# PecanProject/sipnet

Measured on AMD Instinct MI355X. Metric: ensemble-site-timesteps/sec, higher is better.
Workload: dtype f64; 1 GPU; c10k: 1 site(s) x 10240 members per GPU x 17520 half-hourly steps, perturbed params, default flags; sites_per_gpu=1, fast_math=True, gather=n/a (1 GPU), parallelism=ensemble-sharded x1, ranks_seen=1, devices_seen=1, kernel=stepCoopKernel<double, true, true, false>

## Files before the change

### sipnet_amd/csrc/coop_wave_carbon.inc

```

  COOP_CODE_PHASE(0);
  const R K_invLcsw = (R)(1.0 / PRM(leafCSpWt));
  const R K_wtr = (R)PRM(woodTurnoverRate), K_ltr = (R)PRM(leafTurnoverRate);
  const R K_frt = (R)PRM(fineRootTurnoverRate), K_crt = (R)PRM(coarseRootTurnoverRate);
  const R K_la = (R)PRM(leafAllocation), K_wa = (R)PRM(woodAllocation);
  const R K_fa = (R)PRM(fineRootAllocation), K_ca = (R)PRM(coarseRootAllocation);
  const double gddLeafOn = PRM(gddLeafOn);
  const double leafOffDay = PRM(leafOffDay) > 0 ? PRM(leafOffDay) : 1e300;

  const R G_iLeafCN = NCyc ? (R)(1.0 / PRM(leafCN)) : R(0), G_iWoodCN = NCyc ? (R)(1.0 / PRM(woodCN)) : R(0);
  const R G_iFineCN = NCyc ? (R)(1.0 / PRM(fineRootCN)) : R(0), G_resorbC = NCyc ? (R)PRM(leafNResorptionFrac) : R(0);
  const double G_nVolD = NCyc ? PRM(nVolatilizationFrac) : 0.0, G_nLeachD = NCyc ? PRM(nLeachingFrac) : 0.0;
  double plantWoodC = ST(plantWoodC), plantLeafC = ST(plantLeafC), soilC = NCyc ? 0.0 : ST(soilC);
  double coarseRootC = ST(coarseRootC), fineRootC = ST(fineRootC);
  const R X_growthFrac = F_growthResp ? (R)PRM(growthRespFrac) : R(0);
  const R X_lbrK = F_litterPool ? (R)(PRM(litterBreakdownRate) / PRM(baseSoilResp)) : R(0);
  const R X_flr = Opt ? (R)PRM(fracLitterRespired) : R(0), X_1mFlr = Opt ? (R)(1.0 - PRM(fracLitterRespired)) : R(0);
  const R X_soilCH4 = F_anaerobic ? (R)PRM(soilMethaneRate) : R(0);
  const R X_litCH4 = (F_anaerobic && F_litterPool) ? (R)PRM(litterMethaneRate) : R(0);
  const R X_iSoilCSat = (Opt && F_carbonSat) ? (R)(1.0 / PRM(soilCSaturation)) : R(0);
  double litterC = Opt ? ST(litterC) : 0.0;
  auto optSoilSide = [&](R eSoilC, R eLitter, R soilCNow, R fSoil, R qSoilT, R mK, R rootLoss, R aboveLitter, R len,
                         R& rSoil, R& rHet, double& soilGain, double& litterGain, R& methane) {
#pragma clang fp contract(off)
    rSoil = eSoilC * fSoil;
    const R breakdown = eLitter * (X_lbrK * fSoil);
    const R rLitter = breakdown * X_flr, litterToSoil = breakdown * X_1mFlr;
    const R qm = qSoilT * mK;
    const R soilMethane = X_soilCH4 * eSoilC * qm, litterMethane = X_litCH4 * eLitter * qm;
    const R sat = clip01(soilCNow * X_iSoilCSat);
    const R soilInputs = rootLoss + litterToSoil;
    const R dLitter = aboveLitter + soilInputs * sat - litterToSoil - rLitter - litterMethane;
    const R dSoilTwo = soilInputs * (R(1) - sat) - rSoil - soilMethane;
    const R dSoilOne = rootLoss + aboveLitter - rSoil - soilMethane;
// ... 64 lines not shown
                     fineRootCreation * G_iFineCN);
    const R nDemand = plantNDemand();
    postD(&mailPlant[t & 1][0][lane], 0, (double)leafLitter);
    postD(&mailPlant[t & 1][0][lane], 1, (double)woodLitter);
    postD(&mailPlant[t & 1][0][lane], 2, (double)fineRootLoss);
    postD(&mailPlant[t & 1][0][lane], 3, (double)coarseRootLoss);
    postD(&mailPlant[t & 1][0][lane], 4, (double)nDemand);
    postD(&mailPlant[t & 1][0][lane], 5, (double)reductionN);
    postD(&mailPlant[t & 1][0][lane], 6, (double)leafOnN(leafOnCreation + evLeafOnAll));
    postD(&mailPlant[t & 1][0][lane], 7, (double)leafOnN(leafOnCreation));
    postFlag(&seqPlant, t);
    if (__builtin_expect(minNSeq < t, 0)) {
      WAIT_BEGIN()
      takeD1(&mailMinN[t & 1][lane], &seqMinN, t, minNStep);
      WAIT_END(2)
    }
    if (__builtin_expect(__builtin_amdgcn_ballot_w64(!nPlentiful(minNStep, qSoilD, lenD, G_nVolD, G_nLeachD, (double)nDemand)) != 0, 0)) {
      double sAvail, sFixFrac, sUnclaimed;
      takeD3(&mailSupply[0][lane], &seqSupply, t, sAvail, sFixFrac, sUnclaimed);
      const R availableMinN = (R)sAvail, fixFrac = (R)sFixFrac, unclaimed = (R)sUnclaimed;
      const R nUptake = (R(1) - fixFrac) * rmax0(nDemand - unclaimed * invLen);
      const R uptakeDemand = nUptake * len;
      const bool limited = uptakeDemand > R(kTiny) && uptakeDemand > availableMinN;
      const R red = limited ? fdiv(fdiv(availableMinN, R(1) - fixFrac) + unclaimed, nDemand * len) : R(1);
      woodCreation *= red;
      leafCreation *= red;
      fineRootCreation *= red;
      coarseRootCreation *= red;
      postD(&mailDemand[0][lane], 0, (double)plantNDemand());
      postFlag(&seqDemand, t);
    }
  };

  for (int tileStart = curTile * kFastTile; tileStart < tEnd; tileStart += kFastTile, curTile++) {
    if constexpr (Sums) {
      if (tileStart > tBegin) {
        if (RingLds) asm volatile("s_waitcnt vmcnt(0)" ::: "memory");
        else asm volatile("s_waitcnt vmcnt(1)" ::: "memory");
      }
    } else {
    if (tileStart > tBegin) {
      if (RingLds) asm volatile("s_waitcnt vmcnt(1)" ::: "memory");
      else asm volatile("s_waitcnt vmcnt(2)" ::: "memory");
    }
    }
    stageTile(curTile + 1, (curTile + 1) & 1);
    const int tFirst = tileStart > tBegin ? tileStart : tBegin;
    const int tLast = (tileStart + kFastTile) < tEnd ? (tileStart + kFastTile) : tEnd;
    const unsigned char* recB = lds + (curTile & 1) * kTileBytes +
                                (int)(tFirst - tileFirst(curTile)) * (int)sizeof(FastRec);
    int t = tFirst;
    if (!Full && ringClean && !(a.options & SIPNET_KOPT_NO_REGULAR_TILES)) {
      d2 h0, h7;
      i4 hj;
      double hW1, hEndGdd, hEndDay;
      int hTile;
      asm volatile("ds_read_b128 %0, %7\n\tds_read_b128 %1, %7 offset:112\n\tds_read_b128 %2, %7 offset:128\n\t"
                   "ds_read_b64 %3, %7 offset:144\n\tds_read_b32 %4, %7 offset:208\n\tds_read_b64 %5, %7 offset:216\n\t"
                   "ds_read_b64 %6, %7 offset:224\n\ts_waitcnt lgkmcnt(0)"
                   : "=&v"(h0), "=&v"(h7), "=&v"(hj), "=&v"(hW1), "=&v"(hTile), "=&v"(hEndGdd), "=&v"(hEndDay)
                   : "v"(ldsAddr(recB)) : "memory");
      const int tileBits = uni(hTile);
      const bool phenSafe = (allOn || hEndGdd < minGddOn) && (allOff || hEndDay < minOffDay);
      if ((tileBits & FAST_TILE_REGULAR) && __builtin_amdgcn_ballot_w64(!phenSafe) == 0) {
        const R len = (R)h0.x, invLen = (R)h0.y;
        const int nOps = uni(hj.x) >> 16;
        const int slots0 = uni(hj.y);
        auto nextSlot = [](int s) { return s + 1 == SIPNET_RING_SLOTS ? 0 : s + 1; };
        const double wA = nOps == 2 ? h7.y : 0.0, wB = nOps == 2 ? hW1 : h7.y;
        int readSlot = nOps == 2 ? ((slots0 >> 8) & 255) : (slots0 & 255);
        int insSlot = uni(hj.z);
        double vPrev = 0.0;
        if (nOps == 2) {
          const int s0 = slots0 & 255;
          vPrev = RingLds ? ringL[s0 * 64 + lane] : (s0 == lastIns ? lastNpp : (double)ringp[(uint32_t)s0 * ncu]);
        }
        R photosynthesis = 0, rSoil = 0, rVeg = 0, rCoarseRoot = 0, rFineRoot = 0, rHet = 0;
        [[maybe_unused]] R methaneReg = 0;
        double soilGain = 0.0, litterGain = 0.0, ringNew = 0.0;
        R rvN = 0;
        bool rootsOk = true, useLast = false, dyingStep = false;
        auto finishStep = [&](auto mayDie) {
#pragma clang fp contract(off)
          constexpr bool MayDie = decltype(mayDie)::value;
          bool diedNow = false;
          double deathToSoil0 = 0.0, deathToSoil1 = 0.0;
          if (MayDie) ringClean = false;
          if (MayDie && !(rootsOk && (plantWoodC + delta > kTiny))) {
            aliveC = false;
            diedNow = true;
            if (diedAt < 0) diedAt = t;
            deathToSoil0 = fineRootC + coarseRootC;
            deathToSoil1 = plantWoodC + plantLeafC + delta;
            if (NCyc) {
              postD(&mailDeath[0][lane], 0, deathToSoil0);
              postD(&mailDeath[0][lane], 1, deathToSoil1);
              postD(&mailDeath[0][lane], 2, fineRootC * (double)G_iFineCN + coarseRootC * (double)G_iWoodCN);
              postD(&mailDeath[0][lane], 3, plantWoodC * (double)G_iWoodCN + plantLeafC * (double)G_iLeafCN);
            }
            plantWoodC = 0.0;
            plantLeafC = 0.0;
            coarseRootC = 0.0;
            fineRootC = 0.0;
            delta = 0.0;
            ringSum = 0.0;
          }
          plantWoodC = rmax0(plantWoodC);
          plantLeafC = rmax0(plantLeafC);
          coarseRootC = rmax0(coarseRootC);
          fineRootC = rmax0(fineRootC);
          const R tGpp = photosynthesis * len;
          const R tRa = ffma(rVeg, len, (rCoarseRoot + rFineRoot) * len);
          if (NCyc) postD(&mailPend[t & 1][0][lane], 0, (double)(tGpp - tRa));
          postAlive(&mailAlive[(t + 1) & 1][lane], t + 1, diedNow);
          if (!NCyc) {
            soilC += soilGain;
            if (Opt) litterC += litterGain;
            if (MayDie && diedNow) {
              soilC += deathToSoil0;
              if (Opt && F_litterPool) litterC += deathToSoil1;
              else soilC += deathToSoil1;
            }
            soilC = rmax0(soilC);
            if (Opt) litterC = rmax0(litterC);
          }
          const R tRh = (Opt ? rHet : rSoil) * len;
          const R tNee = R(-1.0) * ((tGpp - tRa) - tRh);
          if (!NCyc) totNee += (double)tNee;
          const double npp = (double)(photosynthesis - rVeg - rCoarseRoot - rFineRoot);
          if (!RingLds) asm volatile("s_waitcnt vmcnt(0)" : "+v"(rvN) :: "memory");
          const double vNew = RingLds ? ringNew : (useLast ? lastNpp : (double)rvN);
          if (!(MayDie && diedNow)) {
            ringSum = ffma(-wA, vPrev, ringSum);
            ringSum = ffma(-wB, vNew, ringSum);
            ringSum = ffma(npp, (double)len, ringSum);
          } else {
            ringValidFrom = t + 1;
          }
          vPrev = vNew;
          if (RingLds) {
            ringL[insSlot * 64 + lane] = npp;
          } else {
            ringp[(uint32_t)insSlot * ncu] = (R)npp;
            lastIns = insSlot;
            lastNpp = npp;
          }
          if constexpr (Sums && !NCyc) {
            sumsC.nee += (double)tNee;
            if (--sumsC.left == 0) {
              *oNee = (OutT)sumsC.nee;
              oNee += ldNee;
              sumsC.nee = 0.0;
              sumsC.left = a.sumEvery;
            }
          } else {
          if (!NCyc) {
            *oNee = tNee;
            oNee += ldNee;
          }
          }
          if (__builtin_expect(stageOn, 0)) postRaw(&stage[0][(t - tBegin) & (2 * kStageR - 1)][lane], tNee);
        };
        unsigned dayMask = ((unsigned)tileBits >> 16) >> (t - tileStart);
        for (; t < tLast; t++, dayMask >>= 1) {
#pragma clang fp contract(off)
          MARK("C regular step begin")
          R g1, g2, qSoilT, gFine, gCoarse, moistEff;
          R mK = 0;
          ringNew = 0.0;
          double minNStep = 0.0;
          int minNSeq = 0;
          {
            WAIT_BEGIN()
            if (NCyc)
              takeFactorsN(&mailFac[t & 1][0][lane], &seqFac, &mailMinN[t & 1][lane], &seqMinN, t, g1, g2, gFine, gCoarse,
                           moistEff, minNStep, minNSeq);
            else if (Opt && RingLds)
              takeFactorsRing7(&mailFac[t & 1][0][lane], seqFacMoist, ldsAddr(&ringL[readSlot * 64 + lane]), t, g1,
                               g2, qSoilT, gFine, gCoarse, moistEff, mK, ringNew);
            else if (Opt)
              takeFactors7(&mailFac[t & 1][0][lane], seqFacMoist, t, g1, g2, qSoilT, gFine, gCoarse, moistEff, mK);
            else if (RingLds)
              takeFactorsRing(&mailFac[t & 1][0][lane], seqFacMoist, ldsAddr(&ringL[readSlot * 64 + lane]), t, g1,
                              g2, qSoilT, gFine, gCoarse, moistEff, ringNew);
            else
              takeFactors(&mailFac[t & 1][0][lane], seqFacMoist, t, g1, g2, qSoilT, gFine, gCoarse, moistEff);
            WAIT_END(0)
          }
          const R fSoil = NCyc ? R(0) : qSoilT * moistEff;
          rvN = 0;
          if (!RingLds) {
            if (sizeof(R) == 8)
              asm volatile("global_load_dwordx2 %0, %1, off" : "=&v"(rvN) : "v"(ringp + (uint32_t)readSlot * ncu) : "memory");
            else
              asm volatile("global_load_dword %0, %1, off" : "=&v"(rvN) : "v"(ringp + (uint32_t)readSlot * ncu) : "memory");
          }
          useLast = readSlot == lastIns;
          const bool isDay = (dayMask & 1u) != 0;

          const R eLeaf = (R)plantLeafC, eSoilC = (R)soilC;
          const R eCoarse = (R)coarseRootC, eFine = (R)fineRootC;
          const R totalWoodC = (R)(plantWoodC + delta);
          const R meanNpp = (R)(ringSum * 0.2);
          const R folResp = eLeaf * g1;
          rVeg = ffma(totalWoodC, g2, folResp);
          if (Ext) rVeg += rmax0(X_growthFrac * meanNpp);
          rCoarseRoot = eCoarse * gCoarse;
          rFineRoot = eFine * gFine;
          if (!Opt) rSoil = eSoilC * fSoil;
          const R woodLitter = totalWoodC * K_wtr;
          const R leafLitter = eLeaf * K_ltr;
          R leafCreation = meanNpp * K_la, woodCreation = meanNpp * K_wa;
          const R coarseRootLoss = K_crt * eCoarse, fineRootLoss = K_frt * eFine;
          R coarseRootCreation = K_ca * meanNpp, fineRootCreation = K_fa * meanNpp;
          {
            const R leafDeficit = ffma(eLeaf, invLen, leafCreation) - leafLitter;
            const R ld = rminv(leafDeficit, R(0));
            woodCreation += ld;
            leafCreation -= ld;
            const R fineDef = ffma(eFine, invLen, fineRootCreation) - fineRootLoss;
            const R coarseDef = ffma(eCoarse, invLen, coarseRootCreation) - coarseRootLoss;
            const bool fNeg = fineDef < R(0), cNeg = coarseDef < R(0);
            const R shift = (fNeg != cNeg) ? (fNeg ? fineDef : -coarseDef) : R(0);
            coarseRootCreation += shift;
            fineRootCreation -= shift;
          }
          if (NCyc)
            plantSideN(t, len, invLen, minNStep, minNSeq, (double)moistEff, (double)h0.x, leafLitter, woodLitter, fineRootLoss,
                       coarseRootLoss, R(0), R(0), leafCreation, woodCreation, fineRootCreation, coarseRootCreation);
          accum(plantLeafC, leafCreation - leafLitter, len);
          post(&mailLai[(t + 1) & 1][lane], &seqLai, (R)rmax0(plantLeafC) * K_invLcsw, t + 1);
          accum(plantWoodC, woodCreation - woodLitter, len);
          accum(coarseRootC, coarseRootCreation - coarseRootLoss, len);
          accum(fineRootC, fineRootCreation - fineRootLoss, len);
          if (Opt)
            optSoilSide(eSoilC, (R)litterC, eSoilC, fSoil, qSoilT, mK, coarseRootLoss + fineRootLoss, woodLitter + leafLitter, len,
                        rSoil, rHet, soilGain, litterGain, methaneReg);
          else if (!NCyc) soilGain = (double)((coarseRootLoss + fineRootLoss + woodLitter + leafLitter - rSoil) * len);
          const R r_a = rVeg + rFineRoot + rCoarseRoot;
          const R alloc = leafCreation + woodCreation + fineRootCreation + coarseRootCreation;
          rootsOk = (plantWoodC > kTiny) && (fineRootC + coarseRootC > kTiny);
          photosynthesis = 0;
          if (__builtin_expect(isDay, 0)) {
            WAIT_BEGIN()
            photosynthesis = take(&mailPsn[t & 1][lane], &seqPsn, t);
            WAIT_END(1)
          }
          accum(delta, (photosynthesis - r_a) - alloc, len);
          const bool dies = !(rootsOk && (plantWoodC + delta > kTiny));
          if (__builtin_expect(__builtin_amdgcn_ballot_w64(dies) != 0, 0)) {
            dyingStep = true;
            break;
          }
          finishStep(std::false_type{});
          readSlot = nextSlot(readSlot);
          insSlot = nextSlot(insSlot);
          MARK("C regular step end")
        }
        if (dyingStep) {
          finishStep(std::true_type{});
          t++;
        }
        recB += (int)(t - tFirst) * (int)sizeof(FastRec);
      }
    }
  for (; t < tLast; t++, recB += sizeof(FastRec)) {
#pragma clang fp contract(off)
    d2 q0, q6, q7;
    i4 j0;
    R g1, g2, qSoilT, gFine, gCoarse, moistEff;
    R mK = 0;
    int facSeq, moistSeq;
    double minNStep = 0.0;
    if (Opt) {
      WAIT_BEGIN()
      const unsigned fac = ldsAddr(&mailFac[t & 1][0][lane]);
      const unsigned mst = ldsAddr(&mailFac[t & 1][5][lane]);
      WAIT_DO {
        if (sizeof(R) == 8) {
          asm volatile("ds_read_b128 %0, %13\n\tds_read_b128 %1, %13 offset:96\n\tds_read_b128 %2, %13 offset:112\n\t"
                       "ds_read_b128 %3, %13 offset:128\n\tds_read_b32 %4, %14\n\t"
                       "ds_read_b64 %5, %15\n\tds_read_b64 %6, %15 offset:512\n\tds_read_b64 %7, %15 offset:1024\n\t"
                       "ds_read_b64 %8, %15 offset:1536\n\tds_read_b64 %9, %15 offset:2048\n\t"
                       "ds_read_b32 %10, %16\n\tds_read_b64 %11, %17\n\tds_read_b64 %12, %17 offset:512\n\ts_waitcnt lgkmcnt(0)"
                       : "=&v"(q0), "=&v"(q6), "=&v"(q7), "=&v"(j0), "=&v"(facSeq), "=&v"(g1), "=&v"(g2),
                         "=&v"(qSoilT), "=&v"(gFine), "=&v"(gCoarse), "=&v"(moistSeq), "=&v"(moistEff), "=&v"(mK)
                       : "v"(ldsAddr(recB)), "v"(ldsAddr(&seqFac)), "v"(fac), "v"(ldsAddr(&seqMoist)), "v"(mst)
                       : "memory");
        } else {
          asm volatile("ds_read_b128 %0, %13\n\tds_read_b128 %1, %13 offset:96\n\tds_read_b128 %2, %13 offset:112\n\t"
                       "ds_read_b128 %3, %13 offset:128\n\tds_read_b32 %4, %14\n\t"
                       "ds_read_b32 %5, %15\n\tds_read_b32 %6, %15 offset:256\n\tds_read_b32 %7, %15 offset:512\n\t"
                       "ds_read_b32 %8, %15 offset:768\n\tds_read_b32 %9, %15 offset:1024\n\t"
                       "ds_read_b32 %10, %16\n\tds_read_b32 %11, %17\n\tds_read_b32 %12, %17 offset:256\n\ts_waitcnt lgkmcnt(0)"
                       : "=&v"(q0), "=&v"(q6), "=&v"(q7), "=&v"(j0), "=&v"(facSeq), "=&v"(g1), "=&v"(g2),
                         "=&v"(qSoilT), "=&v"(gFine), "=&v"(gCoarse), "=&v"(moistSeq), "=&v"(moistEff), "=&v"(mK)
// ... 30 lines not shown
        }
      } WAIT_WHILE(uni(facSeq) < t, 26, t);
      qSoilT = 0;
      WAIT_END(0)
    } else {
      WAIT_BEGIN()
      const unsigned fac = ldsAddr(&mailFac[t & 1][0][lane]);
      const unsigned mst = ldsAddr(&mailFac[t & 1][5][lane]);
      WAIT_DO {
        if (sizeof(R) == 8) {
          asm volatile("ds_read_b128 %0, %12\n\tds_read_b128 %1, %12 offset:96\n\tds_read_b128 %2, %12 offset:112\n\t"
                       "ds_read_b128 %3, %12 offset:128\n\tds_read_b32 %4, %13\n\t"
                       "ds_read_b64 %5, %14\n\tds_read_b64 %6, %14 offset:512\n\tds_read_b64 %7, %14 offset:1024\n\t"
                       "ds_read_b64 %8, %14 offset:1536\n\tds_read_b64 %9, %14 offset:2048\n\t"
                       "ds_read_b32 %10, %15\n\tds_read_b64 %11, %16\n\ts_waitcnt lgkmcnt(0)"
                       : "=&v"(q0), "=&v"(q6), "=&v"(q7), "=&v"(j0), "=&v"(facSeq), "=&v"(g1), "=&v"(g2),
                         "=&v"(qSoilT), "=&v"(gFine), "=&v"(gCoarse), "=&v"(moistSeq), "=&v"(moistEff)
                       : "v"(ldsAddr(recB)), "v"(ldsAddr(&seqFac)), "v"(fac), "v"(ldsAddr(&seqMoist)), "v"(mst)
                       : "memory");
        } else {
          asm volatile("ds_read_b128 %0, %12\n\tds_read_b128 %1, %12 offset:96\n\tds_read_b128 %2, %12 offset:112\n\t"
                       "ds_read_b128 %3, %12 offset:128\n\tds_read_b32 %4, %13\n\t"
                       "ds_read_b32 %5, %14\n\tds_read_b32 %6, %14 offset:256\n\tds_read_b32 %7, %14 offset:512\n\t"
                       "ds_read_b32 %8, %14 offset:768\n\tds_read_b32 %9, %14 offset:1024\n\t"
                       "ds_read_b32 %10, %15\n\tds_read_b32 %11, %16\n\ts_waitcnt lgkmcnt(0)"
                       : "=&v"(q0), "=&v"(q6), "=&v"(q7), "=&v"(j0), "=&v"(facSeq), "=&v"(g1), "=&v"(g2),
                         "=&v"(qSoilT), "=&v"(gFine), "=&v"(gCoarse), "=&v"(moistSeq), "=&v"(moistEff)
                       : "v"(ldsAddr(recB)), "v"(ldsAddr(&seqFac)), "v"(fac), "v"(ldsAddr(&seqMoist)), "v"(mst)
                       : "memory");
        }
      } WAIT_WHILE(uni(facSeq) < t || uni(moistSeq) < t, 27, t);
      WAIT_END(0)
    }
    const R fSoil = qSoilT * moistEff;
    const double* rare = (const double*)(recB + 144);
    const int32_t* rareI = (const int32_t*)(recB + 184);
    CSTAMP(0)
    const R len = (R)q0.x, invLen = (R)q0.y;
    const int bits = uni(j0.x);
    const int slots = uni(j0.y);
    const int insSlot = uni(j0.z);
    const int nEv = uni(j0.w);
    const int evSlot0 = slots & 255, evSlot1 = (slots >> 8) & 255;
    R rv0 = 0, rv1 = 0;
    if (!RingLds) {
      if (sizeof(R) == 8)
        asm volatile("global_load_dwordx2 %0, %2, off\n\tglobal_load_dwordx2 %1, %3, off"
                     : "=&v"(rv0), "=&v"(rv1)
                     : "v"(ringp + (uint32_t)evSlot0 * ncu), "v"(ringp + (uint32_t)evSlot1 * ncu) : "memory");
      else
        asm volatile("global_load_dword %0, %2, off\n\tglobal_load_dword %1, %3, off"
                     : "=&v"(rv0), "=&v"(rv1)
                     : "v"(ringp + (uint32_t)evSlot0 * ncu), "v"(ringp + (uint32_t)evSlot1 * ncu) : "memory");
    }
    const bool useLast0 = evSlot0 == lastIns, useLast1 = evSlot1 == lastIns;

    const bool alive0 = aliveC;
    const R eWood = (R)plantWoodC, eLeaf = (R)plantLeafC, eSoilC = (R)soilC;
    const R eCoarse = (R)coarseRootC, eFine = (R)fineRootC;
    const R eLitter = (R)litterC;
    const R totalWoodC = (R)(plantWoodC + delta);
    double preC = 0.0;
    if (wantDiag) preC = (plantWoodC + delta) + plantLeafC + fineRootC + coarseRootC + soilC + (Opt && F_litterPool ? litterC : 0.0);
    R recLeafOffComputed = 0, recEvLeafOn = 0, recEvLeafOnFromWood = 0, recEvLeafOffLitter = 0;
    R evInC = 0, evOutC = 0;
    [[maybe_unused]] R evInN = 0, evOutN = 0;
// ... 330 lines not shown
    const R tRa = ffma(rVeg, len, (rCoarseRoot + rFineRoot) * len);
    const R tNee = R(-1.0) * ((tGpp - tRa) - tRh);
    if (!NCyc) totNee += (double)tNee;
    R tRAbove = 0, tRRoot = 0, tRSoil = 0, tRtot = 0, tNpp = 0;
    if (Full) {
      if (bits & FAST_TRACK_NEW_YEAR) yGpp = yRtot = yRa = yRh = yNpp = yNee = 0.0;
      tRAbove = rVeg * len;
      tRRoot = (rCoarseRoot + rFineRoot) * len;
      tRSoil = tRRoot + tRh;
      tRtot = tRa + tRh;
      tNpp = tGpp - tRa;
      yGpp += (double)tGpp;
      yRa += (double)tRa;
      yRh += (double)tRh;
      yRtot += (double)tRtot;
      yNpp += (double)tNpp;
      yNee += (double)tNee;
      totRa += (double)tRa;
      totRh += (double)tRh;
      totRtot += (double)tRtot;
      totNpp += (double)tNpp;
      yLitter += (double)(leafLitter + recEvLeafOffLitter);
    }

    const double npp = (double)(photosynthesis - rVeg - rCoarseRoot - rFineRoot);
    const double recMeanNpp = Full ? ringSum / 5.0 : 0.0;
    CSTAMP(5)
    {
      if (!RingLds) asm volatile("s_waitcnt vmcnt(0)" : "+v"(rv0), "+v"(rv1) :: "memory");
      const double v0 = RingLds ? ringL[evSlot0 * 64 + lane] : (useLast0 ? lastNpp : (double)rv0);
      const int nOps = bits >> 16;
      if (__builtin_expect(ringClean && insSlot >= 0 && nOps <= 2, 1)) {
        const double v1 = RingLds ? ringL[evSlot1 * 64 + lane] : (useLast1 ? lastNpp : (double)rv1);
        ringSum = ffma(-q7.y, v0, ringSum);
        ringSum = ffma(-rare[0], v1, ringSum);
        ringSum = ffma(npp, (double)len, ringSum);
      } else if (alive) {
        if (insSlot < 0) {
          ringSum = npp * 5.0;
        } else {
          double w0v = v0, w1v = RingLds ? ringL[evSlot1 * 64 + lane] : (useLast1 ? lastNpp : (double)rv1);
          if (ringValidFrom > 0) {
            if (uni(rareI[0]) < ringValidFrom) w0v = 0.0;
            if (uni(rareI[1]) < ringValidFrom) w1v = 0.0;
          }
          ringSum = ffma(-q7.y, w0v, ringSum);
          ringSum = ffma(-rare[0], w1v, ringSum);
          for (int k = 2; k < nOps; k++) {
            const RingOp& op = a.ringOps[opBase + uni(rareI[2]) + k];
            const int os = uni(op.slot);
            const double rvk = RingLds ? ringL[os * 64 + lane]
                                       : (os == lastIns ? lastNpp : (double)ringp[(uint32_t)os * ncu]);
            const double v = (uni(op.insStep) >= ringValidFrom) ? rvk : 0.0;
            ringSum = ffma(-op.w, v, ringSum);
          }
          ringSum = ffma(npp, (double)len, ringSum);
        }
      } else {
        ringValidFrom = t + 1;
      }
    }
    const int insEff = insSlot < 0 ? 0 : insSlot;
    if (RingLds) {
      ringL[insEff * 64 + lane] = npp;
    } else {
      ringp[(uint32_t)insEff * ncu] = (R)npp;
// ... 38 lines not shown
      r[37 * L] = (double)(leafOnFromWood * len);
      r[38 * L] = (double)(recLeafOffComputed * len);
      r[39 * L] = (double)(recEvLeafOn * len);
      r[40 * L] = (double)(recEvLeafOnFromWood * len);
      r[41 * L] = deathWood;
      r[42 * L] = deathRoot;
      r[43 * L] = diedNow ? 1.0 : 0.0;
      recp += (int64_t)SIPNET_NREC * L;
    }
    if constexpr (Sums && !NCyc) {
      sumsC.nee += (double)tNee;
      if (--sumsC.left == 0) {
        *oNee = (OutT)sumsC.nee;
        oNee += ldNee;
        sumsC.nee = 0.0;
        sumsC.left = a.sumEvery;
      }
    } else {
    if (!NCyc) {
      *oNee = tNee;
      oNee += ldNee;
    }
    }
    if (__builtin_expect(stageOn, 0)) postRaw(&stage[0][(t - tBegin) & (2 * kStageR - 1)][lane], tNee);
    CSTAMP(6)
  }
  }
  if constexpr (Sums && !NCyc) {
    if (sumsC.left != a.sumEvery) *oNee = (OutT)sumsC.nee;
  }

  CSTAMP_STORE()
  WAIT_STORE(8)
  if (a.statsPart) {
    asm volatile("s_waitcnt vmcnt(0)" ::: "memory");
    asm volatile("ds_write_b32 %0, %1" :: "v"(ldsAddr(&seqDone[0])), "v"(1) : "memory");
  }
  if (act) {
    if (RingLds)
      for (int k = 0; k < SIPNET_RING_SLOTS; k++) ringp[(uint32_t)k * ncu] = (R)ringL[k * 64 + lane];
    ST(plantWoodC) = plantWoodC;
    ST(plantLeafC) = plantLeafC;
    if (!NCyc) ST(soilC) = soilC;
    if (Opt) ST(litterC) = litterC;
    ST(coarseRootC) = coarseRootC;
    ST(fineRootC) = fineRootC;
    ST(plantCAccountingDelta) = delta;
    ST(ringSum) = ringSum;
    if (!NCyc) ST(totNee) = totNee;
    ST(phenBits) = (double)phenBits;
    ST(ringValidFrom) = (double)ringValidFrom;
    ST(diedAt) = (double)diedAt;
    if (Full) {
      ST(totRa) = totRa;
      ST(totNpp) = totNpp;
      ST(yearlyGpp) = yGpp;
      ST(yearlyRa) = yRa;
      ST(yearlyNpp) = yNpp;
      ST(yearlyLitter) = yLitter;
      if (!NCyc) {
        ST(totRtot) = totRtot;
        ST(totRh) = totRh;
        ST(yearlyRtot) = yRtot;
        ST(yearlyRh) = yRh;
        ST(yearlyNee) = yNee;
      }
// ... 10 lines not shown
```

### sipnet_amd/csrc/coop_wave_light.inc

```

  if (role == 2) {
#pragma clang fp contract(off)
    COOP_CODE_PHASE(2);
    const double leafCSpWt = PRM(leafCSpWt);
    const double convK = kCWeight * (1.0 / kTen9) * (leafCSpWt / PRM(cFracLeaf)) * kSecPerDay;
    const double respPerGram = PRM(baseFolRespFrac) * PRM(aMax);
    const R K_g = (R)((PRM(aMax) * PRM(aMaxFrac) + respPerGram) * convK);
    const R K_tmin = (R)PRM(psnTMin), K_tmax = (R)PRM(psnTMax);
    const R K_invDen = (R)(1.0 / (((PRM(psnTMax) - PRM(psnTMin)) / 2.0) * ((PRM(psnTMax) - PRM(psnTMin)) / 2.0)));
    const R K_slope = (R)PRM(dVpdSlope), K_vexp = (R)PRM(dVpdExp);
    const R K_attl = (R)(-PRM(attenuation) * (1.0 / 6.0) * kLog2e);
    const R K_invHalf = (R)(1.0 / PRM(halfSatPar));
    const R K_frozThr = (R)PRM(frozenSoilThreshold);
    const R K_lgVeg = (R)log2(PRM(vegRespQ10)), K_lgSoil = (R)log2(PRM(soilRespQ10));
    const R K_lgFine = (R)log2(PRM(fineRootQ10)), K_lgCoarse = (R)log2(PRM(coarseRootQ10));
    const R K_fol = (R)((PRM(baseFolRespFrac) * PRM(aMax)) *
                        (kCWeight * (1.0 / kTen9) * (PRM(leafCSpWt) / PRM(cFracLeaf)) * kSecPerDay) *
                        (1.0 / PRM(leafCSpWt)) * exp2(-(PRM(psnTOpt) / 10.0) * log2(PRM(vegRespQ10))));
    const R K_frozFolEff = (R)PRM(frozenSoilFolREff);
    const R K_bvr = (R)PRM(baseVegResp), K_bsr = (R)PRM(baseSoilResp);
    const R K_bfr = (R)PRM(baseFineRootResp), K_bcr = (R)PRM(baseCoarseRootResp);
    R qSoil = 0, gFine = 0, gCoarse = 0;
    bool haveQ = false;
    WAIT_DECL()
    __builtin_amdgcn_s_waitcnt(0);
    for (int tileStart = curTile * kFastTile; tileStart < tEnd; tileStart += kFastTile, curTile++) {
      if (tileStart > tBegin) asm volatile("s_waitcnt vmcnt(0)" ::: "memory");
      stageTile(curTile + 1, (curTile + 1) & 1);
      const int tFirst = tileStart > tBegin ? tileStart : tBegin;
      const int tLast = (tileStart + kFastTile) < tEnd ? (tileStart + kFastTile) : tEnd;
      const unsigned char* recB = lds + (curTile & 1) * kTileBytes +
                                  (int)(tFirst - tileFirst(curTile)) * (int)sizeof(FastRec);
      for (int t = tFirst; t < tLast; t++, recB += sizeof(FastRec)) {
        d2 q1, q2, q3, q5;
        double q6x;
        int bitsV;
// ... 60 lines not shown
```

### sipnet_amd/csrc/step_coop.hip

```cpp
#include <hip/hip_runtime.h>

#include <cstdio>
#include <type_traits>

#include "fast_math.h"
#include "step_kernel.h"

namespace sipnet {
#ifdef SIPNET_COOP_BOUNDED
namespace bounded {
#endif
#ifdef SIPNET_COOP_SUMS_TU
namespace sums2 {
#endif
namespace {

constexpr int kTileBytes = kFastTile * (int)sizeof(FastRec);

#ifdef SIPNET_COOP_BOUNDED
__device__ unsigned long long g_coopStuck[2];
__shared__ int g_coopPoison;
constexpr int kSpinBudget = 1 << 22;
__device__ __forceinline__ bool spinOut(int& n, int id, int step) {
  n++;
// ... 15 lines not shown
#define WAIT_DO do
#define WAIT_WHILE(cond, id, step) while (cond)
#endif

__device__ __forceinline__ void post(double* slot, int* flag, double v, int step) {
  asm volatile("ds_write_b64 %0, %1\n\tds_write_b32 %2, %3"
               :: "v"((unsigned)(size_t)slot), "v"(v), "v"((unsigned)(size_t)flag), "v"(step) : "memory");
}
__device__ __forceinline__ void post(float* slot, int* flag, float v, int step) {
  asm volatile("ds_write_b32 %0, %1\n\tds_write_b32 %2, %3"
               :: "v"((unsigned)(size_t)slot), "v"(v), "v"((unsigned)(size_t)flag), "v"(step) : "memory");
}
__device__ __forceinline__ double take(const double* slot, const int* flag, int step) {
  double v;
  int f;
  WAIT_DO {
    asm volatile("ds_read_b32 %0, %2\n\tds_read_b64 %1, %3\n\ts_waitcnt lgkmcnt(0)"
                 : "=&v"(f), "=&v"(v) : "v"((unsigned)(size_t)flag), "v"((unsigned)(size_t)slot) : "memory");
  } WAIT_WHILE(uni(f) < step, 1, step);
  return v;
}
__device__ __forceinline__ float take(const float* slot, const int* flag, int step) {
  float v;
  int f;
  WAIT_DO {
    asm volatile("ds_read_b32 %0, %2\n\tds_read_b32 %1, %3\n\ts_waitcnt lgkmcnt(0)"
                 : "=&v"(f), "=&v"(v) : "v"((unsigned)(size_t)flag), "v"((unsigned)(size_t)slot) : "memory");
  } WAIT_WHILE(uni(f) < step, 2, step);
  return v;
}
typedef double d2_t __attribute__((ext_vector_type(2)));
typedef int i4_t __attribute__((ext_vector_type(4)));
__device__ __forceinline__ unsigned ldsAddr(const void* p) { return (unsigned)(size_t)p; }
template <class R>
__device__ __forceinline__ R q10Arg(R t10, R lg) {
  R x = t10 * lg;
  asm volatile("" : "+v"(x));
  return x;
}
__device__ __forceinline__ int aliveWord(int step, bool died) { return died ? -(step + 2) : (step + 2); }
__device__ __forceinline__ void postAlive(int* slot, int step, bool died) {
  asm volatile("ds_write_b32 %0, %1" :: "v"((unsigned)(size_t)slot), "v"(aliveWord(step, died)) : "memory");
}
__device__ __forceinline__ void takePgp(const double* slot, const int* flag, const int* alive, int step,
                                        double& pgp, bool& died) {
  int f, w;
  WAIT_DO {
    asm volatile("ds_read_b32 %0, %3\n\tds_read_b64 %1, %4\n\tds_read_b32 %2, %5\n\ts_waitcnt lgkmcnt(0)"
                 : "=&v"(f), "=&v"(pgp), "=&v"(w)
                 : "v"((unsigned)(size_t)flag), "v"((unsigned)(size_t)slot), "v"((unsigned)(size_t)alive) : "memory");
  } WAIT_WHILE(uni(f) < step || uni(w < 0 ? -w : w) < step + 2, 3, step);
  died = w < 0;
}
__device__ __forceinline__ void takePgp(const float* slot, const int* flag, const int* alive, int step,
                                        float& pgp, bool& died) {
  int f, w;
  WAIT_DO {
    asm volatile("ds_read_b32 %0, %3\n\tds_read_b32 %1, %4\n\tds_read_b32 %2, %5\n\ts_waitcnt lgkmcnt(0)"
                 : "=&v"(f), "=&v"(pgp), "=&v"(w)
                 : "v"((unsigned)(size_t)flag), "v"((unsigned)(size_t)slot), "v"((unsigned)(size_t)alive) : "memory");
  } WAIT_WHILE(uni(f) < step || uni(w < 0 ? -w : w) < step + 2, 4, step);
  died = w < 0;
}
typedef double d2v __attribute__((ext_vector_type(2)));
typedef float f2v __attribute__((ext_vector_type(2)));
typedef int i2v __attribute__((ext_vector_type(2)));
// ... 269 lines not shown
#ifdef SIPNET_PH_F
  if (role == 3) return SIPNET_PH_F;
#endif
  if (Sums && sizeof(R) == 8 && NP == 1 && RingLds && !NCyc && !Ext && (role == 0 || role == 1)) return 3;
  if (role == 0) {
    if (NCyc) return 0;
    if (Ext) return 7;
    if (NP == 2) return 2;
    if (NP == 1 && RingLds) return Full ? 4 : 6;
    return 0;
  }
  if (role == 1) {
    if (NCyc) return 0;
    if (Ext) return 1;
    if (NP == 2) return 4;
    if (NP == 1 && RingLds) return Full ? 5 : 6;
    return 0;
  }
  if (role == 2) return (NP == 1 && RingLds && !Full && !NCyc && !Ext) ? 3 : 0;
  if (role == 3) return (NCyc && NP == 1) ? 4 : 0;
  if (role != 4) return 0;
#ifdef SIPNET_PAD_NOPS
  return SIPNET_PAD_NOPS;
#else
  constexpr bool f64 = sizeof(R) == 8;
  if (NCyc) return 4;
  if (Ext) return 4;
  if (NP == 4) return f64 ? 6 : 3;
  if (NP == 2) return Full ? 0 : f64 ? 4 : 7;
  if (!RingLds) return 0;
  return (Full || f64) ? 3 : 4;
#endif
}

template <bool On>
struct CoopSums {
  double nee = 0.0, et = 0.0, gpp = 0.0;
  int left = 0;
};
template <>
struct CoopSums<false> {};
template <class R, bool PlainExp, bool RingLds, bool Full, int NP, bool NCyc = false, bool Ext = false, bool Sums = false, bool PairDiag = false>
__device__ __forceinline__ void coopBody(const FastArgs& a) {
  static_assert(!PairDiag || (NCyc && Full && NP == 2), "PairDiag: the nitrogen cycle's two-chunk full-state layout");
  static_assert(!Sums || !Full, "in-kernel sums: lean launches");
  using OutT = typename std::conditional<Sums, double, R>::type;
  static_assert(!(NP > 1 && RingLds), "two chunks' rings do not fit one CU's LDS");
  static_assert(!NCyc || (NP <= 2 && !RingLds), "nitrogen-cycle layout: one or two chunks, ring in HBM");
  constexpr bool Opt = Ext && !NCyc;
  const bool F_growthResp = Ext && a.flags[SIPNET_F_GROWTH_RESP] != 0, F_leafWater = Ext && a.flags[SIPNET_F_LEAF_WATER] != 0;
  const bool F_flooding = Ext && a.flags[SIPNET_F_FLOODING] != 0, F_carbonSat = Ext && a.flags[SIPNET_F_CARBON_SATURATION] != 0;
  const bool F_litterPool = Opt && a.flags[SIPNET_F_LITTER_POOL] != 0, F_anaerobic = Opt && a.flags[SIPNET_F_ANAEROBIC] != 0;
  constexpr double kNoCap = 3.0e38;
  constexpr bool Pair = NP == 2;
  constexpr bool FacWave = RingLds || (Pair && !NCyc);
#include "coop_mailboxes.inc"
#ifdef SIPNET_NO_STATS
  const bool stageOn = false;
#else
  const bool stageOn = Staged && a.statsPart != nullptr;
#endif
  [[maybe_unused]] const bool firstChunk = blockIdx.x == 0 && sub == 0;
  PROBE_HWID(blockIdx.x * NP + sub, role)
  unsigned char* lds = ldsTilesAll[sub][(role < 0 || role > (NCyc ? 3 : 2)) ? 0 : role];

  const int chunksPerSite = (a.n_members + 63) >> 6;
// ... 470 lines not shown
```

Measured before the change: 21.55 billion ensemble-site-timesteps/s.

## Carry LDS mailbox and ring addresses across steps and post LAI earlier

Adds a carried-tile path for the lean f64 single-chunk LDS-ring variant. Mailbox, alive, factor and ring-slot LDS addresses are kept in registers and advanced by add and subtract flips with explicit wrap points, instead of being recomputed every step. The next-step leaf carbon and LAI are computed and posted right after the factors arrive, so the light wave can proceed sooner. The death check becomes wave ballots, the day bit is tested in place, and fixed s_nop padding is inserted at several points to tune instruction alignment. This adds code complexity, relies on hand-tuned asm and pad counts, and the reordered leaf update must keep the same numerics.

Result: faster. 21.78 billion ensemble-site-timesteps/s, median of 6 (+1.1%).

```diff
diff --git a/sipnet_amd/csrc/coop_wave_carbon.inc b/sipnet_amd/csrc/coop_wave_carbon.inc
--- a/sipnet_amd/csrc/coop_wave_carbon.inc
+++ b/sipnet_amd/csrc/coop_wave_carbon.inc
@@ -1,5 +1,6 @@
 
   COOP_CODE_PHASE(0);
+  constexpr bool Carried = kCoopCarriedTile<R, PlainExp, RingLds, Full, NP, NCyc, Ext, Sums>;
   const R K_invLcsw = (R)(1.0 / PRM(leafCSpWt));
   const R K_wtr = (R)PRM(woodTurnoverRate), K_ltr = (R)PRM(leafTurnoverRate);
   const R K_frt = (R)PRM(fineRootTurnoverRate), K_crt = (R)PRM(coarseRootTurnoverRate);
@@ -130,6 +131,7 @@
     }
   };
 
+  if constexpr (Carried) COOP_CARRIED_PAD(0);
   for (int tileStart = curTile * kFastTile; tileStart < tEnd; tileStart += kFastTile, curTile++) {
     if constexpr (Sums) {
       if (tileStart > tBegin) {
@@ -171,7 +173,33 @@
         double vPrev = 0.0;
         if (nOps == 2) {
           const int s0 = slots0 & 255;
+          if constexpr (Carried)
+            asm volatile("ds_read_b64 %0, %1\n\ts_waitcnt lgkmcnt(0)" : "=&v"(vPrev) : "v"(ldsAddr(&ringL[s0 * 64 + lane])) : "memory");
+          else
           vPrev = RingLds ? ringL[s0 * 64 + lane] : (s0 == lastIns ? lastNpp : (double)ringp[(uint32_t)s0 * ncu]);
+        }
+        [[maybe_unused]] unsigned cFac = 0, cLai = 0, cAlive = 0, cRead = 0, cIns = 0;
+        [[maybe_unused]] unsigned sumFac = 0, sumLai = 0, sumAlive = 0, sumPsnLai = 0;
+        [[maybe_unused]] int cSeq = 0;
+        [[maybe_unused]] int wrapRead = 0, wrapIns = 0, wrapNext = 0;
+        [[maybe_unused]] uint64_t allLanes = 0;
+        if constexpr (Carried) {
+          cFac = ldsAddr(&mailFac[t & 1][0][lane]);
+          sumFac = ldsAddr(&mailFac[0][0][lane]) + ldsAddr(&mailFac[1][0][lane]);
+          cLai = ldsAddr(&mailLai[(t + 1) & 1][lane]);
+          sumLai = ldsAddr(&mailLai[0][lane]) + ldsAddr(&mailLai[1][lane]);
+          cAlive = ldsAddr(&mailAlive[(t + 1) & 1][lane]);
+          sumAlive = ldsAddr(&mailAlive[0][lane]) + ldsAddr(&mailAlive[1][lane]);
+          static_assert(sizeof(mailPsn[0]) == sizeof(mailLai[0]), "mailPsn[t & 1] from mailLai[(t + 1) & 1]: the same slot stride");
+          sumPsnLai = ldsAddr(&mailPsn[1][lane]) + ldsAddr(&mailLai[0][lane]);
+          cSeq = t + 1;
+          asm volatile("" : "+v"(cSeq));
+          cRead = ldsAddr(&ringL[readSlot * 64 + lane]);
+          cIns = ldsAddr(&ringL[insSlot * 64 + lane]);
+          wrapRead = t + (SIPNET_RING_SLOTS - 1 - readSlot);
+          wrapIns = t + (SIPNET_RING_SLOTS - 1 - insSlot);
+          wrapNext = wrapRead < wrapIns ? wrapRead : wrapIns;
+          allLanes = __builtin_amdgcn_ballot_w64(true);
         }
         R photosynthesis = 0, rSoil = 0, rVeg = 0, rCoarseRoot = 0, rFineRoot = 0, rHet = 0;
         [[maybe_unused]] R methaneReg = 0;
@@ -210,7 +238,8 @@
           const R tGpp = photosynthesis * len;
           const R tRa = ffma(rVeg, len, (rCoarseRoot + rFineRoot) * len);
           if (NCyc) postD(&mailPend[t & 1][0][lane], 0, (double)(tGpp - tRa));
-          postAlive(&mailAlive[(t + 1) & 1][lane], t + 1, diedNow);
+          if constexpr (Carried) postAlive(ldsPtr<int>(cAlive), cSeq, diedNow);
+          else postAlive(&mailAlive[(t + 1) & 1][lane], t + 1, diedNow);
           if (!NCyc) {
             soilC += soilGain;
             if (Opt) litterC += litterGain;
@@ -237,7 +266,8 @@
           }
           vPrev = vNew;
           if (RingLds) {
-            ringL[insSlot * 64 + lane] = npp;
+            if constexpr (Carried) postRaw(ldsPtr<double>(cIns), npp);
+            else ringL[insSlot * 64 + lane] = npp;
           } else {
             ringp[(uint32_t)insSlot * ncu] = (R)npp;
             lastIns = insSlot;
@@ -259,8 +289,9 @@
           }
           if (__builtin_expect(stageOn, 0)) postRaw(&stage[0][(t - tBegin) & (2 * kStageR - 1)][lane], tNee);
         };
-        unsigned dayMask = ((unsigned)tileBits >> 16) >> (t - tileStart);
-        for (; t < tLast; t++, dayMask >>= 1) {
+        if constexpr (Carried) COOP_CARRIED_PAD(1);
+        unsigned dayMask = Carried ? ((unsigned)tileBits >> 16) << (tileStart & 16) : ((unsigned)tileBits >> 16) >> (t - tileStart);
+        for (; t < tLast; t++, dayMask >>= Carried ? 0 : 1) {
 #pragma clang fp contract(off)
           MARK("C regular step begin")
           R g1, g2, qSoilT, gFine, gCoarse, moistEff;
@@ -278,12 +309,29 @@
                                g2, qSoilT, gFine, gCoarse, moistEff, mK, ringNew);
             else if (Opt)
               takeFactors7(&mailFac[t & 1][0][lane], seqFacMoist, t, g1, g2, qSoilT, gFine, gCoarse, moistEff, mK);
-            else if (RingLds)
+            else if (RingLds) {
+              if constexpr (Carried)
+                takeFactorsRing(ldsPtr<const R>(cFac), seqFacMoist, cRead, t, g1, g2, qSoilT, gFine, gCoarse, moistEff, ringNew);
+              else
               takeFactorsRing(&mailFac[t & 1][0][lane], seqFacMoist, ldsAddr(&ringL[readSlot * 64 + lane]), t, g1,
                               g2, qSoilT, gFine, gCoarse, moistEff, ringNew);
-            else
+            } else
               takeFactors(&mailFac[t & 1][0][lane], seqFacMoist, t, g1, g2, qSoilT, gFine, gCoarse, moistEff);
             WAIT_END(0)
+          }
+          [[maybe_unused]] R leafLitterFirst = 0, leafCreationFirst = 0, leafDeficitFirst = 0;
+          [[maybe_unused]] double leafNextFirst = 0.0;
+          if constexpr (Carried) {
+            cRead += 512;
+            asm volatile("" : "+v"(cRead));
+            const R leafNow = (R)plantLeafC;
+            leafLitterFirst = leafNow * K_ltr;
+            leafCreationFirst = (R)(ringSum * 0.2) * K_la;
+            leafDeficitFirst = rminv(ffma(leafNow, invLen, leafCreationFirst) - leafLitterFirst, R(0));
+            leafNextFirst = plantLeafC;
+            accum(leafNextFirst, (leafCreationFirst - leafDeficitFirst) - leafLitterFirst, len);
+            post(ldsPtr<R>(cLai), &seqLai, (R)rmax0(leafNextFirst) * K_invLcsw, cSeq);
+            __builtin_amdgcn_sched_barrier(0);
           }
           const R fSoil = NCyc ? R(0) : qSoilT * moistEff;
           rvN = 0;
@@ -294,7 +342,7 @@
               asm volatile("global_load_dword %0, %1, off" : "=&v"(rvN) : "v"(ringp + (uint32_t)readSlot * ncu) : "memory");
           }
           useLast = readSlot == lastIns;
-          const bool isDay = (dayMask & 1u) != 0;
+          const bool isDay = Carried ? (dayMask & (1u << (t & 31))) != 0 : (dayMask & 1u) != 0;
 
           const R eLeaf = (R)plantLeafC, eSoilC = (R)soilC;
           const R eCoarse = (R)coarseRootC, eFine = (R)fineRootC;
@@ -307,13 +355,13 @@
           rFineRoot = eFine * gFine;
           if (!Opt) rSoil = eSoilC * fSoil;
           const R woodLitter = totalWoodC * K_wtr;
-          const R leafLitter = eLeaf * K_ltr;
-          R leafCreation = meanNpp * K_la, woodCreation = meanNpp * K_wa;
+          const R leafLitter = Carried ? leafLitterFirst : eLeaf * K_ltr;
+          R leafCreation = Carried ? leafCreationFirst : meanNpp * K_la, woodCreation = meanNpp * K_wa;
           const R coarseRootLoss = K_crt * eCoarse, fineRootLoss = K_frt * eFine;
           R coarseRootCreation = K_ca * meanNpp, fineRootCreation = K_fa * meanNpp;
           {
             const R leafDeficit = ffma(eLeaf, invLen, leafCreation) - leafLitter;
-            const R ld = rminv(leafDeficit, R(0));
+            const R ld = Carried ? leafDeficitFirst : rminv(leafDeficit, R(0));
             woodCreation += ld;
             leafCreation -= ld;
             const R fineDef = ffma(eFine, invLen, fineRootCreation) - fineRootLoss;
@@ -326,8 +374,9 @@
           if (NCyc)
             plantSideN(t, len, invLen, minNStep, minNSeq, (double)moistEff, (double)h0.x, leafLitter, woodLitter, fineRootLoss,
                        coarseRootLoss, R(0), R(0), leafCreation, woodCreation, fineRootCreation, coarseRootCreation);
-          accum(plantLeafC, leafCreation - leafLitter, len);
-          post(&mailLai[(t + 1) & 1][lane], &seqLai, (R)rmax0(plantLeafC) * K_invLcsw, t + 1);
+          if constexpr (Carried) plantLeafC = leafNextFirst;
+          else accum(plantLeafC, leafCreation - leafLitter, len);
+          if constexpr (!Carried) post(&mailLai[(t + 1) & 1][lane], &seqLai, (R)rmax0(plantLeafC) * K_invLcsw, t + 1);
           accum(plantWoodC, woodCreation - woodLitter, len);
           accum(coarseRootC, coarseRootCreation - coarseRootLoss, len);
           accum(fineRootC, fineRootCreation - fineRootLoss, len);
@@ -337,29 +386,63 @@
           else if (!NCyc) soilGain = (double)((coarseRootLoss + fineRootLoss + woodLitter + leafLitter - rSoil) * len);
           const R r_a = rVeg + rFineRoot + rCoarseRoot;
           const R alloc = leafCreation + woodCreation + fineRootCreation + coarseRootCreation;
-          rootsOk = (plantWoodC > kTiny) && (fineRootC + coarseRootC > kTiny);
+          [[maybe_unused]] uint64_t okMask = 0;
+          if constexpr (Carried)
+            okMask = __builtin_amdgcn_ballot_w64(plantWoodC > kTiny) & __builtin_amdgcn_ballot_w64(fineRootC + coarseRootC > kTiny);
+          else rootsOk = (plantWoodC > kTiny) && (fineRootC + coarseRootC > kTiny);
           photosynthesis = 0;
           if (__builtin_expect(isDay, 0)) {
             WAIT_BEGIN()
-            photosynthesis = take(&mailPsn[t & 1][lane], &seqPsn, t);
+            if constexpr (Carried) COOP_CARRIED_PAD(2);
+            if constexpr (Carried) photosynthesis = take(ldsPtr<const R>(sumPsnLai - cLai), &seqPsn, t);
+            else photosynthesis = take(&mailPsn[t & 1][lane], &seqPsn, t);
             WAIT_END(1)
           }
           accum(delta, (photosynthesis - r_a) - alloc, len);
-          const bool dies = !(rootsOk && (plantWoodC + delta > kTiny));
+          if constexpr (Carried) {
+            okMask &= __builtin_amdgcn_ballot_w64(plantWoodC + delta > kTiny);
+            if (__builtin_expect(okMask != allLanes, 0)) {
+              dyingStep = true;
+              break;
+            }
+          }
+          const bool dies = !Carried && !(rootsOk && (plantWoodC + delta > kTiny));
           if (__builtin_expect(__builtin_amdgcn_ballot_w64(dies) != 0, 0)) {
             dyingStep = true;
             break;
           }
           finishStep(std::false_type{});
+          if constexpr (Carried) {
+            asm volatile("v_sub_u32_e64 %0, %1, %0" : "+v"(cFac) : "v"(sumFac));
+            cLai = sumLai - cLai;
+            asm volatile("" : "+v"(cLai));
+            if (__builtin_expect(t == wrapNext, 0)) {
+              if (t == wrapRead) cRead -= SIPNET_RING_SLOTS * 512;
+              if (t == wrapIns) cIns -= SIPNET_RING_SLOTS * 512;
+              wrapNext = wrapRead > wrapIns ? wrapRead : wrapIns;
+            }
+            cSeq++;
+            cAlive = sumAlive - cAlive;
+            cIns += 512;
+            asm volatile("" : "+v"(cSeq), "+v"(cAlive), "+v"(cIns));
+          } else {
           readSlot = nextSlot(readSlot);
           insSlot = nextSlot(insSlot);
+          }
           MARK("C regular step end")
         }
+        if constexpr (Carried) {
+          int dying = uni((int)dyingStep);
+          asm volatile("" : "+s"(dying));
+          dyingStep = dying != 0;
+        }
         if (dyingStep) {
+          if constexpr (Carried) rootsOk = (plantWoodC > kTiny) && (fineRootC + coarseRootC > kTiny);
           finishStep(std::true_type{});
           t++;
         }
         recB += (int)(t - tFirst) * (int)sizeof(FastRec);
+        if constexpr (Carried) COOP_CARRIED_PAD(3);
       }
     }
   for (; t < tLast; t++, recB += sizeof(FastRec)) {
@@ -456,6 +539,7 @@
       } WAIT_WHILE(uni(facSeq) < t || uni(moistSeq) < t, 27, t);
       WAIT_END(0)
     }
+    if constexpr (Carried) COOP_CARRIED_PAD(4);
     const R fSoil = qSoilT * moistEff;
     const double* rare = (const double*)(recB + 144);
     const int32_t* rareI = (const int32_t*)(recB + 184);
@@ -852,6 +936,7 @@
       const int nOps = bits >> 16;
       if (__builtin_expect(ringClean && insSlot >= 0 && nOps <= 2, 1)) {
         const double v1 = RingLds ? ringL[evSlot1 * 64 + lane] : (useLast1 ? lastNpp : (double)rv1);
+        if constexpr (Carried) COOP_CARRIED_PAD(5);
         ringSum = ffma(-q7.y, v0, ringSum);
         ringSum = ffma(-rare[0], v1, ringSum);
         ringSum = ffma(npp, (double)len, ringSum);
@@ -956,6 +1041,7 @@
 
   CSTAMP_STORE()
   WAIT_STORE(8)
+  if constexpr (Carried) COOP_CARRIED_PAD(6);
   if (a.statsPart) {
     asm volatile("s_waitcnt vmcnt(0)" ::: "memory");
     asm volatile("ds_write_b32 %0, %1" :: "v"(ldsAddr(&seqDone[0])), "v"(1) : "memory");
diff --git a/sipnet_amd/csrc/coop_wave_light.inc b/sipnet_amd/csrc/coop_wave_light.inc
--- a/sipnet_amd/csrc/coop_wave_light.inc
+++ b/sipnet_amd/csrc/coop_wave_light.inc
@@ -2,6 +2,7 @@
   if (role == 2) {
 #pragma clang fp contract(off)
     COOP_CODE_PHASE(2);
+    if constexpr (kCoopCarriedTile<R, PlainExp, RingLds, Full, NP, NCyc, Ext, Sums>) COOP_CARRIED_PAD(7);
     const double leafCSpWt = PRM(leafCSpWt);
     const double convK = kCWeight * (1.0 / kTen9) * (leafCSpWt / PRM(cFracLeaf)) * kSecPerDay;
     const double respPerGram = PRM(baseFolRespFrac) * PRM(aMax);
diff --git a/sipnet_amd/csrc/step_coop.hip b/sipnet_amd/csrc/step_coop.hip
--- a/sipnet_amd/csrc/step_coop.hip
+++ b/sipnet_amd/csrc/step_coop.hip
@@ -71,6 +71,8 @@
 typedef double d2_t __attribute__((ext_vector_type(2)));
 typedef int i4_t __attribute__((ext_vector_type(4)));
 __device__ __forceinline__ unsigned ldsAddr(const void* p) { return (unsigned)(size_t)p; }
+template <class T>
+__device__ __forceinline__ T* ldsPtr(unsigned addr) { return (T*)(size_t)addr; }
 template <class R>
 __device__ __forceinline__ R q10Arg(R t10, R lg) {
   R x = t10 * lg;
@@ -406,6 +408,20 @@
   return (Full || f64) ? 3 : 4;
 #endif
 }
+
+#ifdef SIPNET_COOP_BOUNDED
+constexpr bool kCoopBoundedBuild = true;
+#else
+constexpr bool kCoopBoundedBuild = false;
+#endif
+template <class R, bool PlainExp, bool RingLds, bool Full, int NP, bool NCyc, bool Ext, bool Sums>
+constexpr bool kCoopCarriedTile =
+    !kCoopBoundedBuild && sizeof(R) == 8 && PlainExp && RingLds && !Full && NP == 1 && !NCyc && !Ext && !Sums;
+__device__ constexpr int coopCarriedPad(int where) {
+  constexpr int pad[8] = {1, 3, 2, 2, 1, 1, 4, 4};
+  return pad[where];
+}
+#define COOP_CARRIED_PAD(WHERE) asm volatile(".rept %0\n s_nop 0\n .endr" ::"n"(coopCarriedPad(WHERE)))
 
 template <bool On>
 struct CoopSums {
```
